# levayz/ProtoSAM

Measured on AMD Instinct MI355X. Metric: query-slices/sec (512x512) end-to-end ProtoSAM infer, higher is better.
Workload: dtype f16

## Files before the change

include/protosam_hip.h:

```cpp
#ifndef PROTOSAM_HIP_H
#define PROTOSAM_HIP_H
#include <stddef.h>
#ifdef __cplusplus
extern "C" {
#endif

int psam_gemm_f16(const void* A, const void* W, const float* bias, void* out, const float* resid, const float* gamma,
                  int M, int N, int K, int lda, int ldw, int ldo, int ldr, int resid_mod, int out_seg,
                  int out_seg_stride, int out_seg_off, int epilogue, void* stream);
int psam_gemm_f16_heads(const void* A, const void* W, const float* bias, void* out, int M, int N, int K, int lda, int ldw,
                        int hd, void* stream);
int psam_gemm_f16_ln(const void* A, const void* W, const float* bias, void* out, const float* resid, const float* gamma,
                     int M, int N, int K, int lda, int ldw, int ldo, int ldr, int resid_mod, int out_seg,
                     int out_seg_stride, int out_seg_off, int epilogue, void* out16, int ld16, float* stats,
                     const float* ln_mr, const float* ln_s, void* stream);
int psam_ln_finalize(const float* stats, int M, int D, float eps, float* mr, void* stream);


int psam_gemm_splitk_ranges(int M, int N, int K);
int psam_gemm_f16_splitk_ln(const void* A, const void* W, const float* bias, float* x, int M, int N, int K, int lda, int ldw, int ldx,
                            int ks, float* ws, const float* ln_w, const float* ln_b, float eps, void* out16, int ld16, void* stream);

int psam_gemm_set_tile(int tile);
int psam_gemm_last_tile(int* tile);
int psam_gemm_asm_variant(int variant);
int psam_gemm_set_option(const char* name, int value);
int psam_gemm_set_workspace(void* ptr, size_t bytes);

int psam_layernorm(const float* x, const float* w, const float* b, void* y, float* y2, int M, int D, int ldx, int ldy,
                   float eps, int out_dtype, int zero_tail_rows, void* stream);

int psam_attention_f16(const void* qkv, void* out, const float* rel_h, const float* rel_w, const void* relq,
                       const void* rpack, const void* pad_row, int B, int N, int H, int hd, float scale, int mode, int gh,
                       int gw, int ws, int head_major, void* stream);
int psam_attention_set_variant(int v);
#define PSAM_ATTN_KERNEL_ATTN 1
#define PSAM_ATTN_KERNEL_WATTN 2
#define PSAM_ATTN_KERNEL_WATTN_P 3
#define PSAM_ATTN_KERNEL_GATTN 4
#define PSAM_ATTN_KERNEL_GATTN_ANY 5
#define PSAM_ATTN_KERNEL_ASM_REL 6
#define PSAM_ATTN_KERNEL_ASM_FUSED 7
#define PSAM_ATTN_KERNEL_ASM_NOREL 8
#define PSAM_ATTN_KERNEL_ASM_WINDOW 9
#define PSAM_ATTN_KERNEL_RELPOS 10
#define PSAM_ATTN_KERNEL_FAMILY 0xff
#define PSAM_ATTN_KERNEL_FULL 0x100
// ... 168 lines not shown
```

protosam_amd/_lib.py:

```python
import ctypes
import os

import torch

_HERE = os.path.dirname(os.path.abspath(__file__))
LIB_PATH = os.environ.get("PSAM_LIB_PATH") or os.path.join(_HERE, "libprotosam_hip.so")

c_void_p, c_int, c_float, c_longlong, c_size_t = ctypes.c_void_p, ctypes.c_int, ctypes.c_float, ctypes.c_longlong, ctypes.c_size_t

SIGNATURES = {
    "psam_gemm_f16": [c_void_p, c_void_p, c_void_p, c_void_p, c_void_p, c_void_p] + [c_int] * 12 + [c_void_p],
    "psam_gemm_f16_heads": [c_void_p, c_void_p, c_void_p, c_void_p] + [c_int] * 6 + [c_void_p],
    "psam_gemm_f16_ln": [c_void_p] * 6 + [c_int] * 12 + [c_void_p, c_int, c_void_p, c_void_p, c_void_p, c_void_p],
    "psam_ln_finalize": [c_void_p, c_int, c_int, c_float, c_void_p, c_void_p],
    "psam_gemm_splitk_ranges": [c_int, c_int, c_int],
    "psam_gemm_f16_splitk_ln": [c_void_p, c_void_p, c_void_p, c_void_p] + [c_int] * 7 + [c_void_p, c_void_p, c_void_p, c_float, c_void_p, c_int,
                                c_void_p],
    "psam_gemm_set_tile": [c_int],
    "psam_gemm_last_tile": [ctypes.POINTER(c_int)],
    "psam_gemm_asm_variant": [c_int],
    "psam_gemm_set_option": [ctypes.c_char_p, c_int],
    "psam_gemm_set_workspace": [c_void_p, c_size_t],
    "psam_layernorm": [c_void_p, c_void_p, c_void_p, c_void_p, c_void_p, c_int, c_int, c_int, c_int, c_float,
                       c_int, c_int, c_void_p],
    "psam_attention_f16": [c_void_p, c_void_p, c_void_p, c_void_p, c_void_p, c_void_p, c_void_p, c_int, c_int, c_int, c_int,
                           c_float, c_int, c_int, c_int, c_int, c_int, c_void_p],
    "psam_attention_set_variant": [c_int],
    "psam_attention_last_kernel": [ctypes.POINTER(c_int)],
    "psam_attention_fused_relpos": [c_int] * 6,
    "psam_relpos": [c_void_p, c_void_p, c_void_p, c_void_p, c_void_p] + [c_int] * 7 + [c_float, c_int, c_void_p],
    "psam_alp_bank": [c_void_p, c_int, c_int, c_int, c_int, c_void_p, c_void_p, c_int, c_int, c_int, c_int, c_float, c_float,
                      c_void_p, c_int, c_void_p, c_void_p, c_void_p, c_void_p, c_int, c_void_p],
    "psam_alp_sim": [c_void_p, c_longlong, c_int, c_int, c_int, c_int, c_void_p, c_int, c_void_p, c_float, c_float,
                     c_void_p, c_void_p, c_int, c_void_p],
    "psam_alp_sim_pairs": [c_void_p, c_longlong, c_int, c_int, c_int, c_void_p, c_int, c_int, c_float, c_float, c_void_p, c_void_p,
                           c_void_p],
    "psam_patchify_bilinear": [c_void_p, c_int, c_int, c_int, c_int, c_int, c_int, c_int, c_void_p, c_void_p],
    "psam_bilinear_nchw": [c_void_p, c_int, c_int, c_int, c_int, c_int, c_void_p, c_void_p],
    "psam_resize2d": [c_void_p, c_int, c_int, c_int, c_int, c_int, c_int, c_void_p, c_void_p],
    "psam_bilinear_tokens": [c_void_p, c_longlong, c_int, c_int, c_int, c_int, c_int, c_int, c_int, c_void_p, c_void_p],
    "psam_prob_argmax": [c_void_p, c_int, c_int, c_int, c_int, c_int, c_void_p, c_void_p, c_void_p, c_void_p],
    "psam_broadcast_rows": [c_void_p, c_int, c_void_p, c_int, c_longlong, c_longlong, c_void_p],
# ... 117 lines not shown
```

protosam_amd/csrc/gemm.hip:

```cpp
#include "common.h"
#include "device_tables.h"
#include "gemm_asm_meta.h"
#include <stdlib.h>
#include <string.h>
#include <type_traits>
#include <map>
#include <string>
#include <vector>

enum { EPI_F16 = 0, EPI_GELU_F16 = 1, EPI_F32 = 2, EPI_RELU_F16 = 3 };

struct GemmArgs {
  const half_t* A;
  const half_t* W;
  const float* bias;
  void* out;
  const float* resid;
  const float* gamma;
  int M, N, K;
  int lda, ldw, ldo, ldr;
  int resid_mod;
  int out_seg;
  int out_seg_stride;
  int out_seg_off;
// ... 1029 lines not shown
    (void)hipFuncSetAttribute((const void*)gemm8kp_f16_kernel<EPI_F32, false, true>, hipFuncAttributeMaxDynamicSharedMemorySize, LDS);
    attr = true;
  }
  const int ntm = (p.M + 255) / 256, ntn = p.N / 256;
  GemmArgs q = p;
  q.map_mode = 1;
  KsWorkspace* w = ks_workspace();
  q.ks_ws = w->ptr;
  if (w->used && w->last != s) (void)hipStreamWaitEvent(s, w->done, 0);
  const int total = ntm * ntn * q.ksplit;
  hipLaunchKernelGGL((gemm8kp_f16_kernel<EPI_F32, false, true>), dim3(total < num_cus() ? total : num_cus()), dim3(512), LDS, s, q, total);
  const size_t n4 = (size_t)p.M * (p.N / 4);
  hipLaunchKernelGGL(splitk_reduce_kernel, dim3((unsigned)((n4 + 255) / 256)), dim3(256), 0, s, w->ptr, q.ksplit, p.bias, p.gamma,
                     p.resid, p.ldr, p.resid_mod, reinterpret_cast<float*>(p.out), p.ldo, p.M, p.N);
  if (!w->done) (void)hipEventCreateWithFlags(&w->done, hipEventDisableTiming);
  (void)hipEventRecord(w->done, s);
  w->last = s;
  w->used = true;
}


extern "C" const unsigned char psam_gemm_asm_co[];
extern "C" const unsigned char psam_gemm_asm_co_end[];
struct AsmGemmArgs {
  const void* A; const void* W; const void* bias; void* out; const void* resid; const void* gamma; const void* tab;
  int M, N, K, lda, ldw, ldo, ldr, G, flags, pad;
  void* trace;
  void* out16; float* stats; int ld16, pad2;
};
static_assert(sizeof(AsmGemmArgs) == 128, "kernarg layout of gemm_asm_gen.py");
struct AsmModule { hipModule_t mod = nullptr; int state = 0; std::map<int, std::vector<hipFunction_t>> fns; std::map<std::string, hipFunction_t> named; };
static std::map<int, AsmModule> g_asm;
static int g_asm_variant = 0;
extern "C" int psam_gemm_asm_variant(int v) {
  g_asm_variant = v;
  return PSAM_OK;
}
static AsmModule* asm_module() {
  AsmModule& m = g_asm[psam_current_device()];
  if (m.state == 0) {
    m.state = -1;
    if (hipModuleLoadData(&m.mod, psam_gemm_asm_co) != hipSuccess) { (void)hipGetLastError(); return nullptr; }
    m.state = 1;
  }
  return m.state < 0 ? nullptr : &m;
}
static const hipFunction_t* asm_load(int family = 1) {
  AsmModule* m = asm_module();
  if (!m) return nullptr;
  const int key = family * 1000 + g_asm_variant;
  auto it = m->fns.find(key);
  if (it != m->fns.end()) return it->second.data();
  const char* names[3] = {"f16", "gelu", "f32"};
  const char* suffix1[3] = {"", "_l2", "_ln"};
  const char* suffix3[3] = {"_m16", "_m16", "_ln_m16"};
  const char* const* suffix = family == 3 ? suffix3 : suffix1;
  const int nf = (family != 2 && g_asm_variant == 0) ? 9 : 3;
  std::vector<hipFunction_t> f(9, nullptr);
  for (int i = 0; i < nf; ++i) {
    std::string n = std::string(family == 2 ? "psam_gemm_asm2_" : "psam_gemm_asm_") + names[i % 3] + suffix[i / 3] +
                    (g_asm_variant > 0 ? "_v" + std::to_string(g_asm_variant) : std::string());
    if (hipModuleGetFunction(&f[i], m->mod, n.c_str()) != hipSuccess) {
      (void)hipGetLastError();
      if (i < 6) return nullptr;
      f[i] = nullptr;
    }
  }
  for (int i = nf; i < 6; ++i) f[i] = f[i - 3];
  return (m->fns[key] = f).data();
}
hipFunction_t psam_asm_function(const char* name) {
  AsmModule* m = asm_module();
  if (!m) return nullptr;
  auto it = m->named.find(name);
  if (it != m->named.end()) return it->second;
  hipFunction_t f = nullptr;
  if (hipModuleGetFunction(&f, m->mod, name) != hipSuccess) { (void)hipGetLastError(); f = nullptr; }
  return m->named[name] = f;
}
static bool asm_eligible(const GemmArgs& p, int epilogue, int lnf, int family = 1) {
  if (family == 3 && !asm_load(3)) return false;
  if (lnf) {
    const hipFunction_t* f = asm_load(family);
    const bool cons = p.ln_mr || p.ln_s, prod = p.out16 || p.stats;
    if (!f || g_asm_variant != 0 || (cons && prod)) return false;
    if (cons && (!f[6 + epilogue] || !p.ln_mr || !p.ln_s || !p.bias || (reinterpret_cast<uintptr_t>(p.ln_mr) & 15) || (reinterpret_cast<uintptr_t>(p.ln_s) & 15))) return false;
    if (prod && (!f[8] || !p.out16 || !p.stats)) return false;
  }
  if (p.head_hd || p.out_seg || epilogue > EPI_F32) return false;
  if (p.resid_mod && (epilogue != EPI_F32 || !p.resid || p.resid_mod < 256 || (p.resid_mod & (p.resid_mod - 1)) != 0 || g_asm_variant != 0)) return false;
  if (p.N % 256 || p.K % 64 || p.K < 128 || p.M < 1) return false;
  if ((p.lda % 8) || (p.ldw % 8) || (reinterpret_cast<uintptr_t>(p.A) & 15) || (reinterpret_cast<uintptr_t>(p.W) & 15)) return false;
  const unsigned long long lim = 0xffffffffull;
  if ((unsigned long long)p.M * p.lda * 2 > lim || (unsigned long long)p.N * p.ldw * 2 > lim) return false;
  if (p.bias && (reinterpret_cast<uintptr_t>(p.bias) & 15)) return false;
  if (epilogue == EPI_F32) {
    if ((p.ldo % 4) || (reinterpret_cast<uintptr_t>(p.out) & 15) || (unsigned long long)p.M * p.ldo * 4 > lim) return false;
    if (p.resid && ((p.ldr % 4) || (reinterpret_cast<uintptr_t>(p.resid) & 15) || (unsigned long long)p.M * p.ldr * 4 > lim)) return false;
    if (p.gamma && (reinterpret_cast<uintptr_t>(p.gamma) & 15)) return false;
  } else {
    if (!p.wide16 || (unsigned long long)p.M * p.ldo * 2 > lim) return false;
  }
  return true;
}
static bool asm2_eligible(const GemmArgs& p, int epilogue, int lnf) {
  if (epilogue > EPI_F32 || (p.N % 128)) return false;
  GemmArgs q = p;
  q.N = 256;
  if (lnf || p.resid_mod || !asm_eligible(q, epilogue, 0)) return false;
  if ((unsigned long long)p.N * p.ldw * 2 > 0xffffffffull) return false;
  const int e = epilogue == EPI_F16 ? PSAM_ASM2_E_F16 : epilogue == EPI_GELU_F16 ? PSAM_ASM2_E_GELU : PSAM_ASM2_E_F32;
  return p.K / 64 >= e + 1 && p.K / 64 >= 3;
}
static int launch_asm(const GemmArgs& p, int epilogue, hipStream_t s, int family = 1) {
  const hipFunction_t* fns = asm_load(family);
  if (!fns) return PSAM_ERR_LAUNCH;
  const int ntm = (p.M + 255) / 256, ntn = family == 2 ? p.N / 128 : p.N / 256;
  const PsamDeviceTable* t = psam_device_table(PSAM_TAB_GEMM, {ntm, ntn, pick_map_mode(ntm, ntn), eff_cus()});
  if (!t) return PSAM_ERR_LAUNCH;
  AsmGemmArgs a;
  a.A = p.A; a.W = p.W; a.bias = p.bias; a.out = p.out; a.resid = p.resid; a.gamma = p.gamma; a.tab = t->dev;
  a.M = p.M; a.N = p.N; a.K = p.K; a.lda = p.lda; a.ldw = p.ldw; a.ldo = p.ldo; a.ldr = p.resid ? p.ldr : 0; a.G = t->grid;
  a.flags = p.gamma ? 1 : 0;
  a.pad = (family != 2 && p.resid_mod > 0) ? p.resid_mod - 1 : -1;
  a.trace = nullptr;
  const bool ln_cons = family != 2 && p.ln_mr && p.ln_s, ln_prod = family != 2 && (p.out16 || p.stats);
  if (ln_cons) {
    a.resid = p.ln_mr;
    a.gamma = p.ln_s + p.N;
  }
  a.out16 = p.out16; a.stats = p.stats; a.ld16 = p.ld16; a.pad2 = 0;
  static const char* tr = getenv("PSAM_GEMM_ASM_TRACE");
  const bool trace = tr && g_asm_variant > 0;
  if (trace) { (void)hipMalloc(&a.trace, (size_t)t->grid * 32); (void)hipMemsetAsync(a.trace, 0, (size_t)t->grid * 32, s); }
  size_t sz = ln_prod ? sizeof(a) : 104;
  void* extra[] = {HIP_LAUNCH_PARAM_BUFFER_POINTER, &a, HIP_LAUNCH_PARAM_BUFFER_SIZE, &sz, HIP_LAUNCH_PARAM_END};
  const size_t out_bytes = (size_t)p.M * p.N * (epilogue == EPI_F32 ? 4 : 2);
  const int fsel = (ln_cons || ln_prod) ? 6 + epilogue : epilogue + ((family == 1 && out_bytes <= ((size_t)48 << 20)) ? 3 : 0);
  if (hipModuleLaunchKernel(fns[fsel], t->grid, 1, 1, 256, 1, 1, 0, s, nullptr, extra) != hipSuccess) {
    (void)hipGetLastError();
    return PSAM_ERR_LAUNCH;
  }
  if (trace) {
    std::vector<unsigned> h((size_t)t->grid * 8);
    (void)hipStreamSynchronize(s);
    (void)hipMemcpy(h.data(), a.trace, h.size() * 4, hipMemcpyDeviceToHost);
    (void)hipFree(a.trace);
    double loop = 0, epi = 0, kt = 0, tot = 0, rt = 0;
    unsigned tmax = 0;
    for (int b = 0; b < t->grid; ++b) rt += h[(size_t)t->grid * 4 + b * 4];
    for (int b = 0; b < t->grid; ++b) { loop += h[b * 4]; epi += h[b * 4 + 1]; kt += h[b * 4 + 2]; tot += h[b * 4 + 3]; tmax = h[b * 4 + 3] > tmax ? h[b * 4 + 3] : tmax; }
    const double tiles = kt / (p.K / 64);
    if (kt > 0) fprintf(stderr, "asm%s v%d %dx%dx%d epi%d: %.0f cycles per K-tile, %.0f cycles per epilogue (%.1f tiles per workgroup) kernel entry to exit: mean %.0f max %u cycles = %.1f us (shader clock %.0f MHz)\n", family == 3 ? " m16" : "", g_asm_variant, p.M, p.N,
                        p.K, epilogue, loop / kt, epi / tiles, tiles / t->grid, tot / t->grid, tmax, rt / t->grid * 0.01, rt > 0 ? tot / rt * 100.0 : 0.0);
  }
  return PSAM_OK;
}

#define SKR_MAXV 8
__global__ __launch_bounds__(256) void splitk_reduce_ln_kernel(const float* __restrict__ ws, int ks, const float* __restrict__ bias,
                                                               float* __restrict__ x, int ldx, const float* __restrict__ ln_w,
                                                               const float* __restrict__ ln_b, float eps, half_t* __restrict__ out16, int ld16,
                                                               int M, int N) {
  const int row = blockIdx.x * 4 + (threadIdx.x >> 6), lane = threadIdx.x & 63;
  if (row >= M) return;
  const int nv = N >> 2;
  const size_t Mp = (size_t)((M + 255) & ~255);
  float4 v[SKR_MAXV];
  float* xr = x + (size_t)row * ldx;
#pragma unroll
  for (int k = 0; k < SKR_MAXV; ++k) {
    const int i = lane + 64 * k;
    if (i < nv) v[k] = bias ? reinterpret_cast<const float4*>(bias)[i] : make_float4(0.f, 0.f, 0.f, 0.f);
  }
  for (int r = 0; r < ks; ++r) {
    const float4* pr = reinterpret_cast<const float4*>(ws + ((size_t)r * Mp + row) * N);
// ... 64 lines not shown
  p.M = M; p.N = N; p.K = K; p.lda = lda; p.ldw = ldw; p.ldo = N; p.ldr = 0;
  p.resid_mod = 0; p.out_seg = 0; p.out_seg_stride = 0; p.out_seg_off = 0; p.map_mode = 0; p.head_hd = 0;
  p.out16 = nullptr; p.ld16 = 0; p.stats = nullptr; p.ln_mr = nullptr; p.ln_s = nullptr; p.wide16 = false; p.ksplit = 1; p.ks_ws = nullptr;
  if (!asm_eligible(p, EPI_F32, 0) || (unsigned long long)ks * ((M + 255) & ~255) * N * 4 > 0xffffffffull) return PSAM_ERR_ARG;
  hipFunction_t fn = psam_asm_function("psam_gemm_asm_f32_sk");
  const int ntm = (M + 255) / 256, ntn = N / 256;
  const PsamDeviceTable* t = psam_device_table(PSAM_TAB_SPLITK, {ntm, ntn, pick_map_mode(ntm, ntn), ks, eff_cus()});
  if (!fn || !t) return PSAM_ERR_LAUNCH;
  AsmGemmArgs a;
  a.A = A; a.W = W; a.bias = nullptr; a.out = ws; a.resid = nullptr; a.gamma = nullptr; a.tab = t->dev;
  a.M = M; a.N = N; a.K = K; a.lda = lda; a.ldw = ldw; a.ldo = N; a.ldr = 0; a.G = t->grid; a.flags = 0; a.pad = ks;
  a.trace = nullptr; a.out16 = nullptr; a.stats = nullptr; a.ld16 = 0; a.pad2 = 0;
  size_t sz = 104;
  void* extra[] = {HIP_LAUNCH_PARAM_BUFFER_POINTER, &a, HIP_LAUNCH_PARAM_BUFFER_SIZE, &sz, HIP_LAUNCH_PARAM_END};
  hipStream_t s = (hipStream_t)stream;
  if (hipModuleLaunchKernel(fn, t->grid, 1, 1, 256, 1, 1, 0, s, nullptr, extra) != hipSuccess) {
    (void)hipGetLastError();
    return PSAM_ERR_LAUNCH;
  }
  hipLaunchKernelGGL(splitk_reduce_ln_kernel, dim3((M + 3) / 4), dim3(256), 0, s, ws, ks, bias, x, ldx, ln_w, ln_b, eps, (half_t*)out16, ld16, M, N);
  return psam_launch_status();
}

enum { OPT_ASM = 0, OPT_HALF, OPT_SPLITK, OPT_NSPLIT, OPT_DEEP, OPT_SMALL, OPT_MFMA16, OPT_COUNT };
static const char* const g_opt_names[OPT_COUNT] = {"asm", "half_tiles", "splitk", "nsplit", "deep", "small", "mfma16"};
static const char* const g_opt_env[OPT_COUNT] = {"PSAM_GEMM_ASM", "PSAM_GEMM_HALF", "PSAM_GEMM_SPLITK", "PSAM_GEMM_NSPLIT", "PSAM_GEMM_DEEP", "PSAM_GEMM_SMALL",
                                                 "PSAM_GEMM_MFMA16"};
static int g_opt[OPT_COUNT] = {-1, -1, -1, -1, -1, -1, -1};
static int gemm_option(int i) {
  if (g_opt[i] < 0) { const char* e = getenv(g_opt_env[i]); g_opt[i] = (e && atoi(e) >= 0) ? (atoi(e) != 0) : (i == OPT_MFMA16 ? 2 : 1); }
  return g_opt[i];
}
extern "C" int psam_gemm_set_option(const char* name, int value) {
  if (name && strcmp(name, "max_wgs") == 0) { g_max_wgs = value > 0 ? value : 0; return PSAM_OK; }
  for (int i = 0; i < OPT_COUNT; ++i)
    if (name && strcmp(name, g_opt_names[i]) == 0) { g_opt[i] = (i == OPT_MFMA16 && value < 0) ? 2 : value != 0; return PSAM_OK; }
  return PSAM_ERR_ARG;
}
static int g_last_tile = 0;
extern "C" int psam_gemm_last_tile(int* tile) {
  if (!tile) return PSAM_ERR_ARG;
  *tile = g_last_tile;
  return PSAM_OK;
}
static int g_tile_override = -1;
extern "C" int psam_gemm_set_tile(int t) {
  g_tile_override = t;
  return PSAM_OK;
}
static bool mfma16_auto(int M, int N, int K, int epilogue) {
  const long t256 = (long)((M + 255) / 256) * (N / 256), ncu = eff_cus();
  const size_t out_bytes = (size_t)M * N * (epilogue == EPI_F32 ? 4 : 2);
  return K >= 768 && t256 * 10 >= ncu * 19 && out_bytes > ((size_t)48 << 20);
}
static int pick_tile(int M, int N, int K, int epilogue) {
  if (g_tile_override < 0) {
    const char* e = getenv("PSAM_GEMM_TILE");
    g_tile_override = e ? atoi(e) : 0;
  }
  if (g_tile_override > 0) return g_tile_override;
  if (N % 256 == 0) {
    const long t256 = (long)((M + 255) / 256) * (N / 256);
    const long ncu = eff_cus();
    const long rounds = (t256 + ncu - 1) / ncu;
    const bool short_f32 = epilogue == EPI_F32 && K < 2048;
    const int fill = short_f32 ? 95 : (epilogue == EPI_F32 || rounds > 1) ? 80 : 50;
    if (K >= 768 && t256 * 100 >= rounds * ncu * fill) {
      if (!gemm_option(OPT_ASM)) return 11;
      const int m16 = gemm_option(OPT_MFMA16);
      return (m16 == 1 || (m16 == 2 && mfma16_auto(M, N, K, epilogue))) ? 17 : 15;
    }
  }
  if (N % 128 == 0 && K >= 768) {
    const int half_on = gemm_option(OPT_HALF);
    const long th = (long)((M + 255) / 256) * (N / 128), ncu = eff_cus();
    if (half_on && th * 20 >= ncu * 9) return 16;
// ... 48 lines not shown
  if (ln_cons && (!(epilogue == EPI_F16 || epilogue == EPI_GELU_F16) || !ln.ln_mr || !ln.ln_s)) return PSAM_ERR_ARG;
  const int ntm = (M + BM - 1) / BM, ntn = N / BN;
  dim3 grid(tile_map_grid(ntm, ntn, p.map_mode)), block(256);
  hipStream_t s = (hipStream_t)stream;
  int tsel = epilogue == EPI_RELU_F16 ? 1 : pick_tile(M, N, K, epilogue);
  p.wide16 = (ldo % 8) == 0 && (reinterpret_cast<uintptr_t>(out) & 15) == 0 && (!head_hd || head_hd % 8 == 0);
  if (tsel == 16 && !asm2_eligible(p, epilogue, ln_prod || ln_cons)) tsel = (g_tile_override > 0 || ln_prod || ln_cons) ? 15 : 1;
  if (tsel == 15 && !asm_eligible(p, epilogue, ln_prod || ln_cons)) tsel = (N % 256 == 0) ? 11 : 1;
  if (tsel == 17 && !asm_eligible(p, epilogue, ln_prod || ln_cons, 3)) tsel = (N % 256 == 0) ? 11 : 1;
  if (tsel != 1 && tsel != 11 && tsel != 12 && tsel != 13 && tsel != 15 && tsel != 16 && tsel != 17) tsel = (N % 256 == 0) ? 11 : 1;
  if (tsel == 11 && (N % 256) != 0) tsel = 1;
  if (tsel == 11 && epilogue != EPI_F32 && !p.wide16) tsel = 1;
  if (ln_cons && !p.wide16) return PSAM_ERR_ARG;
  {
    static const bool logging = getenv("PSAM_GEMM_LOG") != nullptr;
    if (logging) {
      static std::map<std::string, int> seen;
      char key[160];
      snprintf(key, sizeof(key), "%d x %d x %d epilogue %d ln %d%d head_hd %d out_seg %d resid_mod %d -> tile %d", M, N, K, epilogue, (int)ln_prod,
               (int)ln_cons, head_hd, out_seg, resid_mod, tsel);
      if (seen[key]++ == 0) fprintf(stderr, "psam_gemm_f16: %s\n", key);
    }
  }
  g_last_tile = tsel;
  if (tsel == 15) return launch_asm(p, epilogue, s);
  if (tsel == 16) return launch_asm(p, epilogue, s, 2);
  if (tsel == 17) return launch_asm(p, epilogue, s, 3);
  p.ksplit = 1;
  p.ks_ws = nullptr;
  {
    const int ks_on = gemm_option(OPT_SPLITK);
    const bool auto_sel = g_tile_override <= 0;
    const KsWorkspace* ksw = ks_workspace();
    hipStreamCaptureStatus cap = hipStreamCaptureStatusNone;
    if (ksw && hipStreamIsCapturing(s, &cap) != hipSuccess) { (void)hipGetLastError(); cap = hipStreamCaptureStatusNone; }
    if (ks_on && auto_sel && ksw && cap == hipStreamCaptureStatusNone && tsel == 1 && epilogue == EPI_F32 && !ln_prod && !ln_cons && !head_hd && N % 256 == 0 &&
        out_seg == 0 && (ldo % 4) == 0) {
      const int t256 = ((M + 255) / 256) * (N / 256), nkt = K / 64;
      int ks = num_cus() / t256;
      if (ks > nkt / 24) ks = nkt / 24;
      if (ks > 8) ks = 8;
      while (ks >= 2 && (size_t)ks * M * N * sizeof(float) > ksw->bytes) --ks;
      if (ks >= 2 && t256 * ks * 4 >= num_cus() * 3) {
        p.ksplit = ks;
        launch8kp_splitk(p, s);
        return psam_launch_status();
// ... 101 lines not shown
```

protosam_amd/csrc/gemm_asm_gen.py:

```python
#!/usr/bin/env python3
import sys

from asm_common import AsmWriter, kernel_begin, kernel_end, kernel_metadata, module_text, younger

GELU_SGPR_CONSTS = [0xb658b1ce, 0xb658b1ce, 0x39bce2fa, 0x39bce2fa, 0xbdd78116, 0xbdd78116, 0xc01354b6, 0xc01354b6]
GELU_C3 = 0x38b90ca2

S_KARG = 0
S_WG = 2
S_A, S_W, S_BIAS, S_OUT, S_RES, S_GAM, S_TAB = 4, 6, 8, 10, 12, 14, 16
S_M, S_N, S_K, S_LDA, S_LDW, S_LDO, S_LDR, S_G, S_FLAGS = 18, 19, 20, 21, 22, 23, 24, 25, 26
S_RMASK = 27
SRD_A, SRD_B, SRD_O, SRD_R, SRD_BIAS, SRD_GAM = 28, 32, 36, 40, 44, 48
S_M0BASE = 68
S_KREM, S_DKREM, S_NK = 69, 70, 71
S_TCUR, S_TDMA, S_TNEXT, S_CUR, S_STRIDE = 72, 73, 74, 75, 76
S_WV, S_WR, S_WC = 77, 78, 79
S_FA, S_FB = 80, 81
S_LDA2, S_LDW2 = 82, 83
S_T0, S_T1, S_T2, S_T3, S_T4 = 84, 85, 86, 87, 88
S_ROW4, S_TOFF, S_N0X4, S_ROFF, S_RROW4 = 89, 90, 91, 92, 93
S_C = 52
S_ROW28, S_RROW28 = 65, 66
S_ACC_LOOP, S_ACC_EPI, S_NKT = 67, 94, 95
S_TS0, S_TS1, S_TRP = 96, 98, 100
S_SKQ, S_SKREM, S_SKR, S_SKT = 96, 97, 98, 99
# ... 363 lines not shown

    def younger(self, vm, tag):
        return younger(vm, tag)

    def epilogue_f16_m16(self, gelu, vm):
        e = self.e
        self.c("---- epilogue (16x16x32 accumulators): bias (+ GELU) -> fp16, through the wave's slab so that 16 lanes store one 256-byte row piece")
        e("s_nop 7")
        e("s_nop 7")
        self.tile_offsets(2)
        e("v_add_u32 v%d, s%d, v%d" % (V_O, S_TOFF, V_OLANE))
        e("s_waitcnt vmcnt(%d)" % self.younger(vm, ("bias", 0)))
        if self.lnc:
            self.c("folded LayerNorm: acc -= mean_row * s_col, one rank-1 MFMA per 16x16 block (fp16 hi / lo operands: fp32-accurate)")
            e("s_waitcnt vmcnt(%d)" % self.younger(vm, ("rs", 0)))
            for rb in range(8):
                for cb in range(8):
                    blk = (rb * 8 + cb) * 4
                    e("v_mfma_f32_16x16x16_f16 a[%d:%d], v[%d:%d], v[%d:%d], a[%d:%d]" % (blk, blk + 3, self.M16_SF + 2 * cb, self.M16_SF + 2 * cb + 1,
                                                                                      self.M16_MF + 2 * rb, self.M16_MF + 2 * rb + 1, blk, blk + 3))
            e("s_nop 7")
            e("s_nop 7")
            e("s_nop 3")
        for rb32 in range(4):
            em = self.F16_EM[rb32 & 1]
            for sub in range(2):
                rb = 2 * rb32 + sub
                for cb in range(8):
                    blk = (rb * 8 + cb) * 4
                    t = V_TMP
                    for i in range(4):
                        e("v_accvgpr_read_b32 v%d, a%d" % (t + i, blk + i))
                    b = self.F16_BIAS + cb * 4
                    if self.lnc:
                        rp, hs = self.M16_RSTD[rb >> 1], rb & 1
                        for hh in range(2):
                            e("v_pk_fma_f32 v[%d:%d], v[%d:%d], v[%d:%d], v[%d:%d] op_sel:[0,%d,0] op_sel_hi:[1,%d,1]" % (
                                t + 2 * hh, t + 2 * hh + 1, t + 2 * hh, t + 2 * hh + 1, rp, rp + 1, b + 2 * hh, b + 2 * hh + 1, hs, hs))
                    else:
                        e("v_pk_add_f32 v[%d:%d], v[%d:%d], v[%d:%d]" % (t, t + 1, t, t + 1, b, b + 1))
                        e("v_pk_add_f32 v[%d:%d], v[%d:%d], v[%d:%d]" % (t + 2, t + 3, t + 2, t + 3, b + 2, b + 3))
                    if gelu:
                        self.gelu_quad(t, self.F16_EM[(rb32 + 1) & 1], t + 2, self.F16_EM[(rb32 + 1) & 1] + 8)
                    e("v_cvt_pk_f16_f32 v%d, v%d, v%d" % (t, t, t + 1))
                    e("v_cvt_pk_f16_f32 v%d, v%d, v%d" % (t + 1, t + 2, t + 3))
                    e("ds_write_b64 v%d, v[%d:%d] offset:%d" % (V_PARK + cb, t, t + 1, sub * 4096))
            for it in range(8):
                e("ds_read_b128 v[%d:%d], v%d offset:%d" % (em + 4 * it, em + 4 * it + 3, V_EADDR + (it & 3), (it >> 2) * 4096))
            for it in range(8):
                e("s_waitcnt lgkmcnt(%d)" % (7 - it))
                e("buffer_store_dwordx4 v[%d:%d], v%d, s[%d:%d], 0 offen%s" % (em + 4 * it, em + 4 * it + 3, V_O, SRD_O, SRD_O + 3, self.sched.get("store_policy", "")))
                e("v_add_u32 v%d, s%d, v%d" % (V_O, S_ROW4, V_O))

    def epilogue_f16(self, gelu, vm):
        if self.m16:
            return self.epilogue_f16_m16(gelu, vm)
        e = self.e
        self.c("---- epilogue: bias (+ GELU) -> fp16, through the wave's slab so that 16 lanes store one 256-byte row piece")
        e("s_nop 7")
        self.tile_offsets(2)
        e("v_add_u32 v%d, s%d, v%d" % (V_O, S_TOFF, V_OLANE))
        e("s_waitcnt vmcnt(%d)" % self.younger(vm, ("bias", 0)))
        if self.lnc:
            self.c("folded LayerNorm: acc -= mean_row * s_col, one rank-1 MFMA per block (fp16 hi / lo operands: fp32-accurate)")
            e("s_waitcnt vmcnt(%d)" % self.younger(vm, ("rs", 0)))
            for rb in range(4):
                for cb in range(4):
                    blk = (rb * 4 + cb) * 16
                    e("v_mfma_f32_32x32x16_f16 a[%d:%d], v[%d:%d], v[%d:%d], a[%d:%d]" % (blk, blk + 15, 96 + 4 * cb, 99 + 4 * cb, 112 + 4 * rb, 115 + 4 * rb, blk, blk + 15))
            e("s_nop 7")
            e("s_nop 7")
            e("s_nop 3")
        for rb in range(4):
            em = self.F16_EM[rb & 1]
            for cb in range(4):
# ... 506 lines not shown
            self.lab("L_pre2_%s" % n)
            self.L += self.pre2_code
            e("s_branch L_pre2_ret_%s" % n)
        self.L += kernel_end(n, 163840, 128 if self.lnp else 104, NUM_SGPR)

    def metadata(self):
        args = ["ptr"] * 7 + ["i32"] * 10 + ["ptr"] + (["ptr"] * 2 + ["i32"] * 2 if self.lnp else [])
        return kernel_metadata(self.name, args, 163840, NUM_SGPR)


def default_sched():
    return {
        "rd23": list(range(16)),
        "tog23": 16,
        "barA": 19,
        "dma": [21 + (5 * p) // 2 for p in range(16)],
        "barB": 46,
        "rd01": [47 + i for i in range(16)],
        "resid_policy": " nt",
        "store_policy": " nt",
    }


def m16_sched(base=None):
    dma = [41 + 5 * p for p in range(16)]
    busy = set(dma) | set(d - 1 for d in dma)
    free = [s for s in range(93, 128) if s not in busy]
    return dict(base or default_sched(), mfma="16x16x32",
                rd1=[1 + 2 * i for i in range(16)],
                tog1=(32, 35), pre_slot=33, barA=36, dma=dma, barB=92,
                rd0=free[:16], adv=free[16])




def variants(trace=False):
    base = default_sched()
    out = [("psam_gemm_asm_f16", EPI_F16, base), ("psam_gemm_asm_gelu", EPI_GELU_F16, base), ("psam_gemm_asm_f32", EPI_F32, base)]
    keep = dict(base, resid_policy="", store_policy="")
    out += [("psam_gemm_asm_f16_l2", EPI_F16, keep), ("psam_gemm_asm_gelu_l2", EPI_GELU_F16, keep), ("psam_gemm_asm_f32_l2", EPI_F32, keep)]
    out += [("psam_gemm_asm_f32_sk", EPI_F32, dict(keep, splitk=True))]
    ln = dict(base, ln_cons=True, ln_prod=True, store16_policy=" nt")
    out += [("psam_gemm_asm_f16_ln", EPI_F16, ln), ("psam_gemm_asm_gelu_ln", EPI_GELU_F16, ln), ("psam_gemm_asm_f32_ln", EPI_F32, ln)]
    out += [("psam_gemm_asm_f16_m16", EPI_F16, m16_sched(base)), ("psam_gemm_asm_gelu_m16", EPI_GELU_F16, m16_sched(base)), ("psam_gemm_asm_f32_m16", EPI_F32, m16_sched(base))]
    out += [("psam_gemm_asm_f16_ln_m16", EPI_F16, m16_sched(ln)), ("psam_gemm_asm_gelu_ln_m16", EPI_GELU_F16, m16_sched(ln)), ("psam_gemm_asm_f32_ln_m16", EPI_F32, m16_sched(ln))]
    if trace:
        traced = dict(base, trace=True)
        for suffix, sc in (("_m16_v1", m16_sched(traced)), ("_v1", traced)):
            out += [("psam_gemm_asm_f16" + suffix, EPI_F16, sc), ("psam_gemm_asm_gelu" + suffix, EPI_GELU_F16, sc), ("psam_gemm_asm_f32" + suffix, EPI_F32, sc)]
    return out


def main():
    trace = "--trace" in sys.argv[1:]
    import gemm_asm2_gen
    l2, meta2, es = gemm_asm2_gen.build_all(trace)
    if "--meta" in sys.argv[1:]:
        out = ["// generated by gemm_asm_gen.py --meta: a half-tile's epilogue is spread over E K-tile iterations of the next one"]
        for nm in ("f16", "gelu", "f32"):
            out.append("#define PSAM_ASM2_E_%s %d" % (nm.upper(), es["psam_gemm_asm2_" + nm]))
        sys.stdout.write("\n".join(out) + "\n")
        return
    ks = variants(trace)
    lines = []
    meta = []
    for name, epi, sc in ks:
        g = Gen(name, epi, sc)
        g.kernel()
        lines += g.L
        meta.append(g.metadata())
    lines += l2
    meta += meta2
    import gattn_asm_gen
    l3, meta3 = gattn_asm_gen.build_all()
    lines += l3
    meta += meta3
    import wattn_asm_gen
# ... 9 lines not shown
```

protosam_amd/ops.py:

```python
import torch

from . import _lib

EPI_F16, EPI_GELU_F16, EPI_F32, EPI_RELU_F16 = 0, 1, 2, 3


_raw_stream = getattr(torch._C, "_cuda_getCurrentRawStream", None)
_raw_device = getattr(torch._C, "_cuda_getDevice", None)


def _stream():
    if _raw_stream is not None and _raw_device is not None:
        return _raw_stream(_raw_device())
    return torch.cuda.current_stream().cuda_stream


class KernelTimer:

    def __init__(self):
        self.records = []
        self.tags = {}

    def start(self):
        e = torch.cuda.Event(enable_timing=True)
# ... 224 lines not shown

DISPATCH_EPOCH = 0


def _bump_dispatch():
    global DISPATCH_EPOCH
    DISPATCH_EPOCH += 1


def dispatch_key():
    return (DISPATCH_EPOCH, QKV_HEAD_MAJOR, FUSE_WINDOW_RELPOS, FUSE_GLOBAL_RELPOS)


def gemm_set_tile(tile):
    _bump_dispatch()
    _lib.check(_lib.lib().psam_gemm_set_tile(int(tile)), "psam_gemm_set_tile")


def gemm_last_tile():
    import ctypes
    t = ctypes.c_int(0)
    _lib.check(_lib.lib().psam_gemm_last_tile(ctypes.byref(t)), "psam_gemm_last_tile")
    return t.value


def gemm_set_option(name, value):
    _bump_dispatch()
    _lib.check(_lib.lib().psam_gemm_set_option(name.encode(), int(value)), "psam_gemm_set_option")


def gemm_asm_variant(v):
    _bump_dispatch()
    _lib.check(_lib.lib().psam_gemm_asm_variant(int(v)), "psam_gemm_asm_variant")


def im2col(x, B, H, W, C, kh, kw, stride, dil, pad, ldo=None, out=None):
    _req(x, torch.float16, "x")
    assert x.is_contiguous()
    Ho = (H + 2 * pad - dil * (kh - 1) - 1) // stride + 1 if stride > 0 else 0
    Wo = (W + 2 * pad - dil * (kw - 1) - 1) // stride + 1 if stride > 0 else 0
    if ldo is None:
        ldo = kh * kw * C
    if out is None:
        if min(B, H, W, C, kh, kw, stride, dil) <= 0 or pad < 0 or Ho <= 0 or Wo <= 0:
            raise ValueError(f"im2col: no output for B={B} {H}x{W}x{C}, kernel {kh}x{kw} stride {stride} dil {dil} pad {pad}")
        out = torch.empty((B * Ho * Wo, ldo), dtype=torch.float16, device=x.device)
# ... 1576 lines not shown
```

Measured before the change: 166.5.

## Pipeline m16 asm GEMM epilogue LDS reads/stores across row-block parking

Adds a new m16 asm GEMM kernel family whose epilogue interleaves the LDS reads and global stores of the previous 32-row slab with the bias/GELU/convert/park work of the current slab, following a fixed schedule plan. It uses an LDS ticket counter to wait only on the needed reads, instead of draining the LDS write/read/store sequence one slab at a time. By default it is enabled only for GELU epilogues with K<=768 when the mfma16 heuristic fires, which targets the MLP up-projection. It adds a separately loaded code object, extra VGPR use for the GELU temporaries, and an env/option toggle.

```diff
diff --git a/include/protosam_hip.h b/include/protosam_hip.h
--- a/include/protosam_hip.h
+++ b/include/protosam_hip.h
@@ -23,6 +23,7 @@
 
 int psam_gemm_set_tile(int tile);
 int psam_gemm_last_tile(int* tile);
+int psam_gemm_last_epi_pipe(int* pipe);
 int psam_gemm_asm_variant(int variant);
 int psam_gemm_set_option(const char* name, int value);
 int psam_gemm_set_workspace(void* ptr, size_t bytes);
diff --git a/protosam_amd/_lib.py b/protosam_amd/_lib.py
--- a/protosam_amd/_lib.py
+++ b/protosam_amd/_lib.py
@@ -18,6 +18,7 @@
                                 c_void_p],
     "psam_gemm_set_tile": [c_int],
     "psam_gemm_last_tile": [ctypes.POINTER(c_int)],
+    "psam_gemm_last_epi_pipe": [ctypes.POINTER(c_int)],
     "psam_gemm_asm_variant": [c_int],
     "psam_gemm_set_option": [ctypes.c_char_p, c_int],
     "psam_gemm_set_workspace": [c_void_p, c_size_t],
diff --git a/protosam_amd/csrc/gemm.hip b/protosam_amd/csrc/gemm.hip
--- a/protosam_amd/csrc/gemm.hip
+++ b/protosam_amd/csrc/gemm.hip
@@ -1075,6 +1075,7 @@
 
 extern "C" const unsigned char psam_gemm_asm_co[];
 extern "C" const unsigned char psam_gemm_asm_co_end[];
+extern "C" const unsigned char psam_gemm_asm_pipe_co[];
 struct AsmGemmArgs {
   const void* A; const void* W; const void* bias; void* out; const void* resid; const void* gamma; const void* tab;
   int M, N, K, lda, ldw, ldo, ldr, G, flags, pad;
@@ -1082,7 +1083,7 @@
   void* out16; float* stats; int ld16, pad2;
 };
 static_assert(sizeof(AsmGemmArgs) == 128, "kernarg layout of gemm_asm_gen.py");
-struct AsmModule { hipModule_t mod = nullptr; int state = 0; std::map<int, std::vector<hipFunction_t>> fns; std::map<std::string, hipFunction_t> named; };
+struct AsmModule { hipModule_t mod = nullptr; hipModule_t mod_pipe = nullptr; int state = 0; std::map<int, std::vector<hipFunction_t>> fns; std::map<std::string, hipFunction_t> named; };
 static std::map<int, AsmModule> g_asm;
 static int g_asm_variant = 0;
 extern "C" int psam_gemm_asm_variant(int v) {
@@ -1107,13 +1108,22 @@
   const char* names[3] = {"f16", "gelu", "f32"};
   const char* suffix1[3] = {"", "_l2", "_ln"};
   const char* suffix3[3] = {"_m16", "_m16", "_ln_m16"};
-  const char* const* suffix = family == 3 ? suffix3 : suffix1;
+  const char* suffix4[3] = {"_m16p", "_m16p", "_ln_m16p"};
+  const char* const* suffix = family == 4 ? suffix4 : family == 3 ? suffix3 : suffix1;
+  const hipFunction_t* f3 = family == 4 ? asm_load(3) : nullptr;
+  if (family == 4 && !f3) return nullptr;
+  if (family == 4 && !m->mod_pipe && hipModuleLoadData(&m->mod_pipe, psam_gemm_asm_pipe_co) != hipSuccess) {
+    (void)hipGetLastError();
+    m->mod_pipe = nullptr;
+    return nullptr;
+  }
   const int nf = (family != 2 && g_asm_variant == 0) ? 9 : 3;
   std::vector<hipFunction_t> f(9, nullptr);
   for (int i = 0; i < nf; ++i) {
+    if (family == 4 && i % 3 == 2) { f[i] = f3[i]; continue; }
     std::string n = std::string(family == 2 ? "psam_gemm_asm2_" : "psam_gemm_asm_") + names[i % 3] + suffix[i / 3] +
                     (g_asm_variant > 0 ? "_v" + std::to_string(g_asm_variant) : std::string());
-    if (hipModuleGetFunction(&f[i], m->mod, n.c_str()) != hipSuccess) {
+    if (hipModuleGetFunction(&f[i], family == 4 ? m->mod_pipe : m->mod, n.c_str()) != hipSuccess) {
       (void)hipGetLastError();
       if (i < 6) return nullptr;
       f[i] = nullptr;
@@ -1131,6 +1141,7 @@
   if (hipModuleGetFunction(&f, m->mod, name) != hipSuccess) { (void)hipGetLastError(); f = nullptr; }
   return m->named[name] = f;
 }
+static int g_last_epi_pipe = 0;
 static bool asm_eligible(const GemmArgs& p, int epilogue, int lnf, int family = 1) {
   if (family == 3 && !asm_load(3)) return false;
   if (lnf) {
@@ -1165,7 +1176,10 @@
   const int e = epilogue == EPI_F16 ? PSAM_ASM2_E_F16 : epilogue == EPI_GELU_F16 ? PSAM_ASM2_E_GELU : PSAM_ASM2_E_F32;
   return p.K / 64 >= e + 1 && p.K / 64 >= 3;
 }
+static bool epi_pipe_wanted(const GemmArgs& p, int epilogue);
 static int launch_asm(const GemmArgs& p, int epilogue, hipStream_t s, int family = 1) {
+  g_last_epi_pipe = family == 3 && epi_pipe_wanted(p, epilogue);
+  if (g_last_epi_pipe) family = 4;
   const hipFunction_t* fns = asm_load(family);
   if (!fns) return PSAM_ERR_LAUNCH;
   const int ntm = (p.M + 255) / 256, ntn = family == 2 ? p.N / 128 : p.N / 256;
@@ -1204,7 +1218,7 @@
     for (int b = 0; b < t->grid; ++b) rt += h[(size_t)t->grid * 4 + b * 4];
     for (int b = 0; b < t->grid; ++b) { loop += h[b * 4]; epi += h[b * 4 + 1]; kt += h[b * 4 + 2]; tot += h[b * 4 + 3]; tmax = h[b * 4 + 3] > tmax ? h[b * 4 + 3] : tmax; }
     const double tiles = kt / (p.K / 64);
-    if (kt > 0) fprintf(stderr, "asm%s v%d %dx%dx%d epi%d: %.0f cycles per K-tile, %.0f cycles per epilogue (%.1f tiles per workgroup) kernel entry to exit: mean %.0f max %u cycles = %.1f us (shader clock %.0f MHz)\n", family == 3 ? " m16" : "", g_asm_variant, p.M, p.N,
+    if (kt > 0) fprintf(stderr, "asm%s v%d %dx%dx%d epi%d: %.0f cycles per K-tile, %.0f cycles per epilogue (%.1f tiles per workgroup) kernel entry to exit: mean %.0f max %u cycles = %.1f us (shader clock %.0f MHz)\n", family == 4 ? " m16p" : family == 3 ? " m16" : "", g_asm_variant, p.M, p.N,
                         p.K, epilogue, loop / kt, epi / tiles, tiles / t->grid, tot / t->grid, tmax, rt / t->grid * 0.01, rt > 0 ? tot / rt * 100.0 : 0.0);
   }
   return PSAM_OK;
@@ -1315,19 +1329,20 @@
   return psam_launch_status();
 }
 
-enum { OPT_ASM = 0, OPT_HALF, OPT_SPLITK, OPT_NSPLIT, OPT_DEEP, OPT_SMALL, OPT_MFMA16, OPT_COUNT };
-static const char* const g_opt_names[OPT_COUNT] = {"asm", "half_tiles", "splitk", "nsplit", "deep", "small", "mfma16"};
+enum { OPT_ASM = 0, OPT_HALF, OPT_SPLITK, OPT_NSPLIT, OPT_DEEP, OPT_SMALL, OPT_MFMA16, OPT_EPI_PIPE, OPT_COUNT };
+static const char* const g_opt_names[OPT_COUNT] = {"asm", "half_tiles", "splitk", "nsplit", "deep", "small", "mfma16", "epi_pipe"};
 static const char* const g_opt_env[OPT_COUNT] = {"PSAM_GEMM_ASM", "PSAM_GEMM_HALF", "PSAM_GEMM_SPLITK", "PSAM_GEMM_NSPLIT", "PSAM_GEMM_DEEP", "PSAM_GEMM_SMALL",
-                                                 "PSAM_GEMM_MFMA16"};
-static int g_opt[OPT_COUNT] = {-1, -1, -1, -1, -1, -1, -1};
+                                                 "PSAM_GEMM_MFMA16", "PSAM_GEMM_EPI_PIPE"};
+static int g_opt[OPT_COUNT] = {-1, -1, -1, -1, -1, -1, -1, -1};
+static bool opt_tristate(int i) { return i == OPT_MFMA16 || i == OPT_EPI_PIPE; }
 static int gemm_option(int i) {
-  if (g_opt[i] < 0) { const char* e = getenv(g_opt_env[i]); g_opt[i] = (e && atoi(e) >= 0) ? (atoi(e) != 0) : (i == OPT_MFMA16 ? 2 : 1); }
+  if (g_opt[i] < 0) { const char* e = getenv(g_opt_env[i]); g_opt[i] = (e && atoi(e) >= 0) ? (atoi(e) != 0) : (opt_tristate(i) ? 2 : 1); }
   return g_opt[i];
 }
 extern "C" int psam_gemm_set_option(const char* name, int value) {
   if (name && strcmp(name, "max_wgs") == 0) { g_max_wgs = value > 0 ? value : 0; return PSAM_OK; }
   for (int i = 0; i < OPT_COUNT; ++i)
-    if (name && strcmp(name, g_opt_names[i]) == 0) { g_opt[i] = (i == OPT_MFMA16 && value < 0) ? 2 : value != 0; return PSAM_OK; }
+    if (name && strcmp(name, g_opt_names[i]) == 0) { g_opt[i] = (opt_tristate(i) && value < 0) ? 2 : value != 0; return PSAM_OK; }
   return PSAM_ERR_ARG;
 }
 static int g_last_tile = 0;
@@ -1336,6 +1351,11 @@
   *tile = g_last_tile;
   return PSAM_OK;
 }
+extern "C" int psam_gemm_last_epi_pipe(int* pipe) {
+  if (!pipe) return PSAM_ERR_ARG;
+  *pipe = g_last_epi_pipe;
+  return PSAM_OK;
+}
 static int g_tile_override = -1;
 extern "C" int psam_gemm_set_tile(int t) {
   g_tile_override = t;
@@ -1345,6 +1365,14 @@
   const long t256 = (long)((M + 255) / 256) * (N / 256), ncu = eff_cus();
   const size_t out_bytes = (size_t)M * N * (epilogue == EPI_F32 ? 4 : 2);
   return K >= 768 && t256 * 10 >= ncu * 19 && out_bytes > ((size_t)48 << 20);
+}
+static bool epi_pipe_auto(int M, int N, int K, int epilogue) {
+  return epilogue == EPI_GELU_F16 && K <= 768 && mfma16_auto(M, N, K, epilogue);
+}
+static bool epi_pipe_wanted(const GemmArgs& p, int epilogue) {
+  if (epilogue != EPI_F16 && epilogue != EPI_GELU_F16) return false;
+  const int o = gemm_option(OPT_EPI_PIPE);
+  return o == 1 || (o == 2 && g_asm_variant == 0 && epi_pipe_auto(p.M, p.N, p.K, epilogue));
 }
 static int pick_tile(int M, int N, int K, int epilogue) {
   if (g_tile_override < 0) {
@@ -1439,6 +1467,7 @@
       if (seen[key]++ == 0) fprintf(stderr, "psam_gemm_f16: %s\n", key);
     }
   }
+  g_last_epi_pipe = 0;
   g_last_tile = tsel;
   if (tsel == 15) return launch_asm(p, epilogue, s);
   if (tsel == 16) return launch_asm(p, epilogue, s, 2);
diff --git a/protosam_amd/csrc/gemm_asm_gen.py b/protosam_amd/csrc/gemm_asm_gen.py
--- a/protosam_amd/csrc/gemm_asm_gen.py
+++ b/protosam_amd/csrc/gemm_asm_gen.py
@@ -1,7 +1,7 @@
 #!/usr/bin/env python3
 import sys
 
-from asm_common import AsmWriter, kernel_begin, kernel_end, kernel_metadata, module_text, younger
+from asm_common import AsmWriter, LdsCounter, kernel_begin, kernel_end, kernel_metadata, module_text, younger
 
 GELU_SGPR_CONSTS = [0xb658b1ce, 0xb658b1ce, 0x39bce2fa, 0x39bce2fa, 0xbdd78116, 0xbdd78116, 0xc01354b6, 0xc01354b6]
 GELU_C3 = 0x38b90ca2
@@ -411,35 +411,91 @@
             e("s_nop 7")
             e("s_nop 7")
             e("s_nop 3")
+        if self.sched.get("epi_pipe"):
+            return self.emit_slabs_m16_pipe(gelu)
         for rb32 in range(4):
             em = self.F16_EM[rb32 & 1]
-            for sub in range(2):
-                rb = 2 * rb32 + sub
-                for cb in range(8):
-                    blk = (rb * 8 + cb) * 4
-                    t = V_TMP
-                    for i in range(4):
-                        e("v_accvgpr_read_b32 v%d, a%d" % (t + i, blk + i))
-                    b = self.F16_BIAS + cb * 4
-                    if self.lnc:
-                        rp, hs = self.M16_RSTD[rb >> 1], rb & 1
-                        for hh in range(2):
-                            e("v_pk_fma_f32 v[%d:%d], v[%d:%d], v[%d:%d], v[%d:%d] op_sel:[0,%d,0] op_sel_hi:[1,%d,1]" % (
-                                t + 2 * hh, t + 2 * hh + 1, t + 2 * hh, t + 2 * hh + 1, rp, rp + 1, b + 2 * hh, b + 2 * hh + 1, hs, hs))
-                    else:
-                        e("v_pk_add_f32 v[%d:%d], v[%d:%d], v[%d:%d]" % (t, t + 1, t, t + 1, b, b + 1))
-                        e("v_pk_add_f32 v[%d:%d], v[%d:%d], v[%d:%d]" % (t + 2, t + 3, t + 2, t + 3, b + 2, b + 3))
-                    if gelu:
-                        self.gelu_quad(t, self.F16_EM[(rb32 + 1) & 1], t + 2, self.F16_EM[(rb32 + 1) & 1] + 8)
-                    e("v_cvt_pk_f16_f32 v%d, v%d, v%d" % (t, t, t + 1))
-                    e("v_cvt_pk_f16_f32 v%d, v%d, v%d" % (t + 1, t + 2, t + 3))
-                    e("ds_write_b64 v%d, v[%d:%d] offset:%d" % (V_PARK + cb, t, t + 1, sub * 4096))
+            for g in range(16):
+                self.park_block_m16(rb32, g, gelu, self.F16_EM[(rb32 + 1) & 1], e)
             for it in range(8):
-                e("ds_read_b128 v[%d:%d], v%d offset:%d" % (em + 4 * it, em + 4 * it + 3, V_EADDR + (it & 3), (it >> 2) * 4096))
+                e(self.emit_read_m16(rb32, it))
             for it in range(8):
                 e("s_waitcnt lgkmcnt(%d)" % (7 - it))
-                e("buffer_store_dwordx4 v[%d:%d], v%d, s[%d:%d], 0 offen%s" % (em + 4 * it, em + 4 * it + 3, V_O, SRD_O, SRD_O + 3, self.sched.get("store_policy", "")))
-                e("v_add_u32 v%d, s%d, v%d" % (V_O, S_ROW4, V_O))
+                self.emit_store_m16(rb32, it)
+
+    def park_block_m16(self, rb32, g, gelu, gt, lds_issue):
+        e = self.e
+        sub, cb = g >> 3, g & 7
+        rb = 2 * rb32 + sub
+        blk = (rb * 8 + cb) * 4
+        t = V_TMP
+        for i in range(4):
+            e("v_accvgpr_read_b32 v%d, a%d" % (t + i, blk + i))
+        b = self.F16_BIAS + cb * 4
+        if self.lnc:
+            rp, hs = self.M16_RSTD[rb >> 1], rb & 1
+            for hh in range(2):
+                e("v_pk_fma_f32 v[%d:%d], v[%d:%d], v[%d:%d], v[%d:%d] op_sel:[0,%d,0] op_sel_hi:[1,%d,1]" % (
+                    t + 2 * hh, t + 2 * hh + 1, t + 2 * hh, t + 2 * hh + 1, rp, rp + 1, b + 2 * hh, b + 2 * hh + 1, hs, hs))
+        else:
+            e("v_pk_add_f32 v[%d:%d], v[%d:%d], v[%d:%d]" % (t, t + 1, t, t + 1, b, b + 1))
+            e("v_pk_add_f32 v[%d:%d], v[%d:%d], v[%d:%d]" % (t + 2, t + 3, t + 2, t + 3, b + 2, b + 3))
+        if gelu:
+            self.gelu_quad(t, gt, t + 2, gt + 8)
+        e("v_cvt_pk_f16_f32 v%d, v%d, v%d" % (t, t, t + 1))
+        e("v_cvt_pk_f16_f32 v%d, v%d, v%d" % (t + 1, t + 2, t + 3))
+        lds_issue("ds_write_b64 v%d, v[%d:%d] offset:%d" % (V_PARK + cb, t, t + 1, sub * 4096))
+
+    def emit_read_m16(self, rb32, it):
+        em = self.F16_EM[rb32 & 1]
+        return "ds_read_b128 v[%d:%d], v%d offset:%d" % (em + 4 * it, em + 4 * it + 3, V_EADDR + (it & 3), (it >> 2) * 4096)
+
+    def emit_store_m16(self, rb32, it):
+        e = self.e
+        em = self.F16_EM[rb32 & 1]
+        e("buffer_store_dwordx4 v[%d:%d], v%d, s[%d:%d], 0 offen%s" % (em + 4 * it, em + 4 * it + 3, V_O, SRD_O, SRD_O + 3, self.sched.get("store_policy", "")))
+        e("v_add_u32 v%d, s%d, v%d" % (V_O, S_ROW4, V_O))
+
+    M16_GT = 212
+
+    def emit_slabs_m16_pipe(self, gelu):
+        e = self.e
+        plan = self.sched["epi_pipe"]
+        assert sorted(plan) == sorted(k + str(it) for k in "rs" for it in range(8))
+        at = dict((p, g) for g, p in enumerate(plan))
+        for it in range(8):
+            assert (at["r%d" % it] >= 8) == (it < 4) and (at["s%d" % it] >= 8) == (it < 4), plan
+            assert at["r%d" % it] < at["s%d" % it], plan
+            assert it in (0, 4) or at["s%d" % (it - 1)] < at["s%d" % it], plan
+        gt = self.M16_GT
+        used = set(range(gt, gt + 4)) | set(range(gt + 8, gt + 12))
+        live = set(range(V_TMP, V_TMP + 12)) | set(range(self.F16_BIAS, self.F16_BIAS + 32)) | set(range(self.F16_EM[0], self.F16_EM[0] + 32))
+        live |= set(range(self.F16_EM[1], self.F16_EM[1] + 32)) | set(range(V_PARK, V_PARK + 16)) | set(range(V_EADDR, V_EADDR + 4))
+        live |= set(r + i for r in self.M16_RSTD for i in range(2)) | set(range(V_SET[0], V_SET[2])) | set(range(0, 25))
+        assert not (used & live), sorted(used & live)
+        assert used <= set(range(self.M16_SF, self.M16_MF + 16))
+        lds = LdsCounter(e)
+        ticket = {}
+        def side(rb32, p):
+            it = int(p[1])
+            if p[0] == "r":
+                ticket[rb32, it] = lds.issue(self.emit_read_m16(rb32, it))
+            else:
+                lds.need(ticket[rb32, it])
+                self.emit_store_m16(rb32, it)
+        for rb32 in range(4):
+            for g in range(16):
+                src = rb32 if g >= 8 else rb32 - 1
+                if src >= 0:
+                    side(src, plan[g])
+                self.park_block_m16(rb32, g, gelu, gt, lds.issue)
+        for p in plan[:8]:
+            if p[0] == "r":
+                side(3, p)
+        for p in plan[:8]:
+            if p[0] == "s":
+                side(3, p)
+        assert sorted(ticket) == [(s, it) for s in range(4) for it in range(8)]
 
     def epilogue_f16(self, gelu, vm):
         if self.m16:
@@ -992,14 +1048,18 @@
     }
 
 
-def m16_sched(base=None):
+EPI_PIPE = ("r4", "r5", "r6", "r7", "s4", "s5", "s6", "s7", "r0", "r1", "r2", "r3", "s0", "s1", "s2", "s3")
+
+
+def m16_sched(base=None, epi_pipe=None):
     dma = [41 + 5 * p for p in range(16)]
     busy = set(dma) | set(d - 1 for d in dma)
     free = [s for s in range(93, 128) if s not in busy]
     return dict(base or default_sched(), mfma="16x16x32",
                 rd1=[1 + 2 * i for i in range(16)],
                 tog1=(32, 35), pre_slot=33, barA=36, dma=dma, barB=92,
-                rd0=free[:16], adv=free[16])
+                rd0=free[:16], adv=free[16],
+                epi_pipe=epi_pipe)
 
 
 
@@ -1021,8 +1081,28 @@
     return out
 
 
+def pipe_variants(trace=False):
+    base = default_sched()
+    ln = dict(base, ln_cons=True, ln_prod=True, store16_policy=" nt")
+    out = [("psam_gemm_asm_f16_m16p", EPI_F16, m16_sched(base, EPI_PIPE)), ("psam_gemm_asm_gelu_m16p", EPI_GELU_F16, m16_sched(base, EPI_PIPE))]
+    out += [("psam_gemm_asm_f16_ln_m16p", EPI_F16, m16_sched(ln, EPI_PIPE)), ("psam_gemm_asm_gelu_ln_m16p", EPI_GELU_F16, m16_sched(ln, EPI_PIPE))]
+    if trace:
+        sc = m16_sched(dict(base, trace=True), EPI_PIPE)
+        out += [("psam_gemm_asm_f16_m16p_v1", EPI_F16, sc), ("psam_gemm_asm_gelu_m16p_v1", EPI_GELU_F16, sc)]
+    return out
+
+
 def main():
     trace = "--trace" in sys.argv[1:]
+    if "--pipe" in sys.argv[1:]:
+        lines, meta = [], []
+        for name, epi, sc in pipe_variants(trace):
+            g = Gen(name, epi, sc)
+            g.kernel()
+            lines += g.L
+            meta.append(g.metadata())
+        sys.stdout.write(module_text(lines, meta))
+        return
     import gemm_asm2_gen
     l2, meta2, es = gemm_asm2_gen.build_all(trace)
     if "--meta" in sys.argv[1:]:
diff --git a/protosam_amd/csrc/gemm_asm_pipe_blob.S b/protosam_amd/csrc/gemm_asm_pipe_blob.S
--- /dev/null
+++ b/protosam_amd/csrc/gemm_asm_pipe_blob.S
@@ -0,0 +1,9 @@
+    .section .rodata
+    .globl psam_gemm_asm_pipe_co
+    .globl psam_gemm_asm_pipe_co_end
+    .balign 4096
+psam_gemm_asm_pipe_co:
+    .incbin "gemm_asm_pipe.co"
+psam_gemm_asm_pipe_co_end:
+    .byte 0
+    .section .note.GNU-stack,"",@progbits
diff --git a/protosam_amd/ops.py b/protosam_amd/ops.py
--- a/protosam_amd/ops.py
+++ b/protosam_amd/ops.py
@@ -270,6 +270,13 @@
     t = ctypes.c_int(0)
     _lib.check(_lib.lib().psam_gemm_last_tile(ctypes.byref(t)), "psam_gemm_last_tile")
     return t.value
+
+
+def gemm_last_epi_pipe():
+    import ctypes
+    t = ctypes.c_int(0)
+    _lib.check(_lib.lib().psam_gemm_last_epi_pipe(ctypes.byref(t)), "psam_gemm_last_epi_pipe")
+    return bool(t.value)
 
 
 def gemm_set_option(name, value):
```

Measured after the change: 166.7, median of 5. No clear change (+0.2%).
